# YangHai-1218/RADet

Hardware: AMD Instinct MI355X
Metric: images/sec train-step, r50_ycbv_pbr 640x480 bs=4/GPU (higher is better)
Workload: dtype f32

## Files before the change

include/radet_hip.h:

```cpp
#ifndef RADET_HIP_H
#define RADET_HIP_H
#include <stdint.h>

#ifdef __cplusplus
extern "C" {
#endif


typedef struct RadetConvDesc {
    const float* w;
    const float* bias;
    const float* bn_gamma;
    const float* bn_beta;
    const float* bn_mean;
    const float* bn_var;
    float* wf;
    float* wft;
    float* bias_f;
    const float* dwf_slabs;
    const float* dbias_partials;
    float* dw;
    float* dbias;
    float* dgamma;
    float* dbeta;
// ... 17 lines not shown
    void* y_amax;
    const void* x1_amax;
    const void* w1_amax;
    void* y1_amax;
    void* yq;
    void* yq_amax;
    const void* x_true_amax;
    const void* w_l1;
    const void* bias_amax;
    const void* addend_amax;
} RadetScales;

int radet_gather_table_rows(int M);
int radet_build_gather_table(int* table, int B, int KH, int KW, int so, int sr, int off, int div, const int* seg_desc,
                             int nseg, void* stream);
enum {
    RADET_TILE_ID_MASK = 0xFF,
    RADET_TILE_SYMBOL = 0x100,
    RADET_TILE_BK32 = 0x200,
    RADET_TILE_MATH_BF16 = 0x400,
    RADET_TILE_STORE_BF16 = 0x800,
    RADET_TILE_SPLITK = 0x1000,
    RADET_TILE_SPLITK_MASK = 0xF000,
    RADET_TILE_OUT_F32 = 0x10000,
    RADET_TILE_STAGES3 = 0x20000,
    RADET_TILE_STAGES4 = 0x40000,
    RADET_TILE_ROWPAIRS = 0x80000,
    RADET_TILE_STREAMK = 0x100000,
    RADET_TILE_STREAMK_MASK = 0x700000,
    RADET_TILE_X3 = 0x1000000,
    RADET_TILE_P3 = 0x2000000,
    RADET_TILE_H2 = 0x8000000,
    RADET_TILE_MASKQ = 0x10000000
};
int radet_conv2d_igemm(const float* x, const float* w, const float* bias, const float* addend, const float* mask,
                       float* y, const int* gather_table, int M, int Cin, int Cout, int KH, int KW, int relu,
                       int tile_override, float* splitk_ws, size_t splitk_ws_floats, void* stream);
int radet_conv2d_igemm_s(const float* x, const float* w, const float* bias, const float* addend, const float* mask,
                         float* y, const int* gather_table, int M, int Cin, int Cout, int KH, int KW, int relu,
                         int tile_override, float* splitk_ws, size_t splitk_ws_floats, void* stream, const RadetScales* sc);
int radet_conv2d_igemm_pair_s(const float* x0, const float* w0, const float* bias0, const float* addend0,
                              const float* mask0, float* y0, const float* x1, const float* w1, const float* bias1,
                              const float* addend1, const float* mask1, float* y1, const int* gather_table, int M,
                              int Cin, int Cout, int KH, int KW, int relu, int tile_override, float* splitk_ws,
                              size_t splitk_ws_floats, void* stream, const RadetScales* sc);
int radet_conv2d_igemm_taps_s(const float* x, const float* w, const float* addend, const float* mask, float* y,
                              const int* gather_table, const int* out_rows, const int* tap_ids_host, int ntaps, int kt_w,
                              int M, int Cin, int Cout, int tile_override, float* splitk_ws, size_t splitk_ws_floats,
                              void* stream, const RadetScales* sc);
int radet_conv2d_igemm_classes_s(const float* x, const float* w, const float* addend, const float* mask, float* y,
                                 const int* gather_table, const int* out_rows, const int* tap_ids_host,
                                 const int* cls_ntaps, const int* cls_start, int ncls, int kt_w, int M, int Cin, int Cout,
                                 int tile_override, float* splitk_ws, size_t splitk_ws_floats, void* stream,
                                 const RadetScales* sc);
int radet_conv2d_igemm_pair(const float* x0, const float* w0, const float* bias0, const float* addend0,
                            const float* mask0, float* y0, const float* x1, const float* w1, const float* bias1,
                            const float* addend1, const float* mask1, float* y1, const int* gather_table, int M, int Cin,
                            int Cout, int KH, int KW, int relu, int tile_override, float* splitk_ws,
                            size_t splitk_ws_floats, void* stream);
int radet_conv2d_igemm_taps(const float* x, const float* w, const float* addend, const float* mask, float* y,
                            const int* gather_table, const int* out_rows, const int* tap_ids_host, int ntaps, int kt_w,
                            int M, int Cin, int Cout, int tile_override, float* splitk_ws, size_t splitk_ws_floats,
                            void* stream);
int radet_conv2d_igemm_classes(const float* x, const float* w, const float* addend, const float* mask, float* y,
                               const int* gather_table, const int* out_rows, const int* tap_ids_host, const int* cls_ntaps,
                               const int* cls_start, int ncls, int kt_w, int M, int Cin, int Cout, int tile_override,
// ... 373 lines not shown
```

radet_amd/csrc/common.h:

```cpp
#pragma once
#include <hip/hip_runtime.h>
#include <stdint.h>

#define RADET_MAX_SEG 8

struct RadetSeg {
    int row_end;
    int row_begin;
    int in_row_off;
    int Hi, Wi, Ho, Wo;
};

struct RadetSegs {
    int nseg;
    RadetSeg s[RADET_MAX_SEG];
};

#define RADET_OK 0
#define RADET_ERR_ARG -1
#define RADET_ERR_LAUNCH -2

static inline int radet_check_launch() {
    hipError_t e = hipGetLastError();
    return e == hipSuccess ? RADET_OK : RADET_ERR_LAUNCH;
// ... 1 lines not shown

typedef float f32x16 __attribute__((ext_vector_type(16)));
typedef float f32x4 __attribute__((ext_vector_type(4)));

__device__ __forceinline__ float wave_sum(float v) {
#pragma unroll
    for (int o = 32; o > 0; o >>= 1) v += __shfl_xor(v, o, 64);
    return v;
}
__device__ __forceinline__ double wave_sum_d(double v) {
#pragma unroll
    for (int o = 32; o > 0; o >>= 1) v += __shfl_xor(v, o, 64);
    return v;
}
__device__ __forceinline__ float wave_max(float v) {
#pragma unroll
    for (int o = 32; o > 0; o >>= 1) v = fmaxf(v, __shfl_xor(v, o, 64));
    return v;
}

template <int BYTES>
__device__ __forceinline__ void radet_kernarg_warm() {
    typedef const char __attribute__((address_space(4))) * kptr_t;
    const kptr_t kp = (kptr_t)__builtin_amdgcn_kernarg_segment_ptr();
    constexpr int N = (BYTES + 63) / 64;
    unsigned d[N];
#pragma unroll
    for (int i = 0; i < N; ++i) asm volatile("s_load_dword %0, %1, %2" : "=s"(d[i]) : "s"(kp), "n"(i * 64));
    asm volatile("s_waitcnt lgkmcnt(0)" ::: "memory");
#pragma unroll
    for (int i = 0; i < N; ++i) asm volatile("" ::"s"(d[i]));
}

__device__ __forceinline__ int xcd_remap(int bid, int nwg) {
    const int q = nwg >> 3, r = nwg & 7;
    const int xcd = bid & 7, k = bid >> 3;
    const int base = xcd < r ? xcd * (q + 1) : r * (q + 1) + (xcd - r) * q;
    return base + k;
}

typedef float rd_f32x2 __attribute__((ext_vector_type(2)));
typedef __bf16 rd_bf16x2 __attribute__((ext_vector_type(2)));
__device__ __forceinline__ unsigned radet_pack_bf16(float lo, float hi) {
    const rd_f32x2 v = {lo, hi};
    return __builtin_bit_cast(unsigned, __builtin_convertvector(v, rd_bf16x2));
}
template <class T> __device__ __forceinline__ float4 ld4(const T* p, size_t i4);
template <> __device__ __forceinline__ float4 ld4<float>(const float* p, size_t i4) {
    return reinterpret_cast<const float4*>(p)[i4];
}
template <> __device__ __forceinline__ float4 ld4<__bf16>(const __bf16* p, size_t i4) {
    const uint2 u = reinterpret_cast<const uint2*>(p)[i4];
    return make_float4(__uint_as_float(u.x << 16), __uint_as_float(u.x & 0xFFFF0000u), __uint_as_float(u.y << 16),
                       __uint_as_float(u.y & 0xFFFF0000u));
}
template <class T> __device__ __forceinline__ void st4(T* p, size_t i4, float4 v);
template <> __device__ __forceinline__ void st4<float>(float* p, size_t i4, float4 v) {
    reinterpret_cast<float4*>(p)[i4] = v;
}
template <> __device__ __forceinline__ void st4<__bf16>(__bf16* p, size_t i4, float4 v) {
    reinterpret_cast<uint2*>(p)[i4] = make_uint2(radet_pack_bf16(v.x, v.y), radet_pack_bf16(v.z, v.w));
}

__host__ __device__ __forceinline__ size_t radet_plane_off(int c) {
    return (size_t)(c >> 5) * 96 + (c & 31);
}
__device__ __forceinline__ void radet_split3(const float4 v, uint2& hi, uint2& mid, uint2& lo) {
    const float x[4] = {v.x, v.y, v.z, v.w};
    unsigned h[4], m[4], l[4];
#pragma unroll
    for (int i = 0; i < 4; ++i) {
        h[i] = __float_as_uint(x[i]) & 0xFFFF0000u;
// ... 103 lines not shown
```

radet_amd/csrc/conv_common.h:

```cpp
#pragma once
#include "common.h"
#include "../../include/radet_hip.h"
#include <stdlib.h>
#include <type_traits>

#define RADET_SPLIT_COUNTERS 16384
#ifndef RADET_P3_DBG
#define RADET_P3_DBG 0
#endif

struct ConvPtrs {
    const float* x;
    const float* w;
    const float* bias;
    const float* addend;
    const float* mask;
    float* y;
    const unsigned* xs;
    const unsigned* ws;
    unsigned* ys;
    _Float16* yq;
    unsigned* yqs;
    const unsigned* xt;
    const unsigned* wl1;
    const unsigned* bs;
    const unsigned* as;
};

struct ConvArgs {
    ConvPtrs p[2];
    int groups;
    const int* rowtab;
    float* partial;
    int* counters;
    const int* out_rows;
    int tap_ids[16];
    int KTw;
    int M, Mp, Cin, Cout, KH, KW;
    int relu;
    int sk, it_per_split;
    int n_full, sk_tail, it_per_tail;
    int io;
    int sk_wgs, sk_base, sk_rem;
    int cls_nt, cls_b[3];
    int dbg;
    int maskq;
};

__device__ __forceinline__ float ld_act(const float* p, size_t o, int io) {
    return io ? (float)reinterpret_cast<const __bf16*>(p)[o] : p[o];
}
__device__ __forceinline__ void st_out(float* p, size_t o, float v, int io) {
    if (io == 1) reinterpret_cast<__bf16*>(p)[o] = (__bf16)v;
    else p[o] = v;
}


typedef const __attribute__((address_space(1))) void* gptr_t;
typedef __attribute__((address_space(3))) void* lptr_t;

#ifndef RADET_BUFLDS
#define RADET_BUFLDS 1
#endif
__device__ __forceinline__ __amdgpu_buffer_rsrc_t radet_rsrc(const void* base) {
    return __builtin_amdgcn_make_buffer_rsrc(const_cast<void*>(base), 0, 0xFFFFFF00u, 0x00020000);
}
#if RADET_BUFLDS
#define radet_lds_load16(base, ok, elem_off, dst) \
    __builtin_amdgcn_raw_ptr_buffer_load_lds(radet_rsrc(base), (dst), 16, \
        (int)((ok) ? (unsigned)((elem_off) * sizeof(*(base))) : 0xFFFFFFFFu), 0, 0, 0)
#else
#define radet_lds_load16(base, ok, elem_off, dst) \
    __builtin_amdgcn_global_load_lds((gptr_t)((ok) ? (const void*)((base) + (elem_off)) : (const void*)(radet_zero_page + (threadIdx.x & 63) * 4)), \
                                     (dst), 16, 0, 0)
#endif

__device__ __forceinline__ void radet_pipe_barrier() {
    asm volatile("s_waitcnt lgkmcnt(0)" ::: "memory");
    __builtin_amdgcn_s_barrier();
// ... 417 lines not shown
    acc1 = __builtin_amdgcn_mfma_f32_32x32x16_f16(al, bh, acc1, 0, 0, 0);
}
struct PairScaleRaw { unsigned xt, wl1, bs, as; };
__device__ __forceinline__ PairScaleRaw igemm_pair_scale_load(const ConvPtrs& P) {
    PairScaleRaw r;
    r.xt = radet_amax_load(P.xt); r.wl1 = radet_amax_load(P.wl1);
    r.bs = P.bs ? radet_amax_load(P.bs) : 0u;
    r.as = P.as ? radet_amax_load(P.as) : 0u;
    return r;
}
__device__ __forceinline__ void igemm_pair_scale(const ConvPtrs& P, PairScaleRaw r, bool store, float& qs, float& qs2) {
    asm volatile("" : "+v"(r.xt), "+v"(r.wl1), "+v"(r.bs), "+v"(r.as));
    float bound = __uint_as_float(radet_amax_reduce(r.xt)) * __uint_as_float(radet_amax_reduce(r.wl1));
    bound += __uint_as_float(radet_amax_reduce(r.bs));
    bound += __uint_as_float(radet_amax_reduce(r.as));
    bound *= 1.0001f;
    const unsigned bits = __float_as_uint(bound);
    if (store && threadIdx.x == 0) radet_amax_store(P.yqs, bits);
    const int e = radet_h2_exp(bits);
    qs = radet_pow2(e);
    qs2 = radet_pow2(e + 11);
}

__device__ __forceinline__ void h2_combine(f32x16& acc0, const f32x16& acc1, float inv_a, float inv_b) {
#pragma unroll
    for (int r = 0; r < 16; ++r) acc0[r] = (fmaf(acc1[r], 1.0f / 2048.0f, acc0[r]) * inv_a) * inv_b;
}

struct TileWord {
    int id;
    int splitk;
    int stages;
    int streamk;
    bool symbol, bk32, math_bf16, store_bf16, out_f32, rowpairs, x3, p3, h2, maskq;
};
inline TileWord decode_tile(int t) {
    TileWord r;
    r.id = t & RADET_TILE_ID_MASK;
    r.splitk = (t & RADET_TILE_SPLITK_MASK) / RADET_TILE_SPLITK;
    r.stages = (t & RADET_TILE_STAGES4) ? 4 : ((t & RADET_TILE_STAGES3) ? 3 : 2);
    r.streamk = (t & RADET_TILE_STREAMK_MASK) / RADET_TILE_STREAMK;
    r.symbol = t & RADET_TILE_SYMBOL; r.bk32 = t & RADET_TILE_BK32;
    r.math_bf16 = t & RADET_TILE_MATH_BF16; r.store_bf16 = t & RADET_TILE_STORE_BF16; r.out_f32 = t & RADET_TILE_OUT_F32;
    r.rowpairs = t & RADET_TILE_ROWPAIRS; r.x3 = t & RADET_TILE_X3; r.p3 = t & RADET_TILE_P3; r.h2 = t & RADET_TILE_H2;
    r.maskq = t & RADET_TILE_MASKQ;
    return r;
}
struct WgradFlags {
    int tile;
    bool math_bf16, store_bf16, one_tap, px32, x3, p3, kdiv4, kdiv2, h2, deep, windows;
};
inline WgradFlags decode_wgrad(int f) {
    WgradFlags r;
    r.tile = (f & RADET_WGRAD_TILE_MASK) / RADET_WGRAD_TILE;
    r.math_bf16 = f & RADET_WGRAD_MATH_BF16; r.store_bf16 = f & RADET_WGRAD_STORE_BF16; r.one_tap = f & RADET_WGRAD_ONE_TAP;
    r.px32 = f & RADET_WGRAD_PX32; r.x3 = f & RADET_WGRAD_X3; r.p3 = f & RADET_WGRAD_P3; r.kdiv4 = f & RADET_WGRAD_KDIV4;
    r.kdiv2 = f & RADET_WGRAD_KDIV2; r.h2 = f & RADET_WGRAD_H2; r.deep = f & RADET_WGRAD_DEEP; r.windows = f & RADET_WGRAD_WINDOWS;
    return r;
}

bool radet_launch_igemm_h2(int choice, const ConvArgs& a, hipStream_t st, int tag, int bk, size_t ws_floats, int stages,
                           bool no_tail_split);
struct WgradArgs;
int radet_launch_wgrad_h2(const WgradArgs& a, const WgradFlags& f, int bm, int bn, hipStream_t st);
```

radet_amd/csrc/conv_igemm.hip:

```cpp
#include "common.h"
#include "../../include/radet_hip.h"
#include <stdlib.h>
#include <type_traits>

#include "conv_common.h"

#include "conv_igemm_kernel.h"
#include "conv_wgrad_kernel.h"

struct PredTile { int base_row, H, W, yx; };
struct PredArgs {
    const float* x;
    const float* w[2];
    const float* bias[2];
    float* y[2];
    int c[2];
    const PredTile* tiles;
    int Cin;
};

__global__ __launch_bounds__(512) void pred3x3_patch_kernel(const PredArgs a) {
    constexpr int TH = 8, TW = 16, PW = TW + 2, PP = (TH + 2) * PW;
    constexpr int PROWS = 192, WROWS = 9 * 32;
    constexpr int A_BYTES = PROWS * 64, BUF_BYTES = (PROWS + WROWS) * 64;
// ... 880 lines not shown
    return radet_conv2d_igemm_classes_s(x, w, addend, mask, y, gather_table, out_rows, tap_ids_host, cls_ntaps, cls_start, ncls,
                                        kt_w, M, Cin, Cout, tile_override, splitk_ws, splitk_ws_floats, stream, nullptr);
}

static int igemm_impl(const float* x, const float* w, const float* bias, const float* addend, const float* mask,
                      float* y, const int* gather_table, int M, int Cin, int Cout, int KH, int KW, int relu,
                      int tile_override, float* splitk_ws, size_t splitk_ws_floats, const int* out_rows,
                      const int* tap_ids, int kt_w, void* stream, const ConvPtrs* second, const int* cls,
                      const RadetScales* sc) {
    const TileWord tw = decode_tile(tile_override);
    const bool h16 = tw.store_bf16;
    const bool p3 = tw.p3 && !h16;
    if (h16 || p3) {
        if (Cin % 32 != 0) return RADET_ERR_ARG;
        Cin /= 2;
    }
    if (Cin % 16 != 0 || Cin <= 0 || Cout <= 0 || M <= 0 || KH * KW > 16 ||
        (gather_table == nullptr && (KH * KW != 1 || out_rows != nullptr || cls != nullptr)))
        return RADET_ERR_ARG;
    ConvArgs a;
    a.io = h16 ? (tw.out_f32 ? 2 : 1) : 0;
    a.out_rows = out_rows;
    for (int t = 0; t < 16; ++t) a.tap_ids[t] = tap_ids ? (t < KH * KW ? tap_ids[t] : 0) : t;
    a.cls_nt = 0; a.cls_b[0] = a.cls_b[1] = a.cls_b[2] = 0x7fffffff;
    if (cls != nullptr) {
        for (int t = 0; t < 16; ++t) a.tap_ids[t] = tap_ids[t];
        for (int c = 0; c < cls[0]; ++c) {
            a.cls_nt |= cls[1 + c] << (4 * c);
            if (c > 0) a.cls_b[c - 1] = cls[5 + c];
        }
    }
    a.KTw = kt_w > 0 ? kt_w : KH * KW;
    { static const int dbg = getenv("RADET_DBG_IGEMM") ? atoi(getenv("RADET_DBG_IGEMM")) : 0; a.dbg = dbg; }
    a.maskq = tw.maskq && mask != nullptr;
    if (a.maskq && (h16 || Cout % 32 != 0 || second != nullptr)) return RADET_ERR_ARG;
    if (y == nullptr && (sc == nullptr || sc->yq == nullptr)) return RADET_ERR_ARG;
    a.p[0].x = x; a.p[0].w = w; a.p[0].bias = bias; a.p[0].addend = addend; a.p[0].mask = mask; a.p[0].y = y;
    a.p[0].xs = sc ? (const unsigned*)sc->x_amax : nullptr;
    a.p[0].ws = sc ? (const unsigned*)sc->w_amax : nullptr;
    a.p[0].ys = sc ? (unsigned*)sc->y_amax : nullptr;
    a.p[0].yq = sc ? (_Float16*)sc->yq : nullptr;
    a.p[0].yqs = sc ? (unsigned*)sc->yq_amax : nullptr;
    a.p[0].xt = sc ? (const unsigned*)sc->x_true_amax : nullptr;
    a.p[0].wl1 = sc ? (const unsigned*)sc->w_l1 : nullptr;
    a.p[0].bs = (sc && bias) ? (const unsigned*)sc->bias_amax : nullptr;
    a.p[0].as = (sc && addend) ? (const unsigned*)sc->addend_amax : nullptr;
    if (a.p[0].yq != nullptr) {
        if (h16 || Cout % 32 != 0 || a.p[0].yqs == nullptr || a.p[0].xt == nullptr || a.p[0].wl1 == nullptr ||
            (bias && a.p[0].bs == nullptr) || (addend && a.p[0].as == nullptr) || second != nullptr)
            return RADET_ERR_ARG;
    }
    a.p[1] = a.p[0];
    a.groups = 1;
    if (second != nullptr) {
        a.p[1] = *second;
        a.p[1].yq = nullptr; a.p[1].yqs = nullptr; a.p[1].xt = a.p[1].wl1 = a.p[1].bs = a.p[1].as = nullptr;
        a.p[1].xs = sc ? (const unsigned*)sc->x1_amax : nullptr;
        a.p[1].ws = sc ? (const unsigned*)sc->w1_amax : nullptr;
        a.p[1].ys = sc ? (unsigned*)sc->y1_amax : nullptr;
        a.groups = 2;
    }
    a.rowtab = gather_table;
    a.Cin = Cin; a.Cout = Cout; a.KH = KH; a.KW = KW;
    a.relu = relu;
    a.M = M;
    a.Mp = radet_gather_table_rows(M);
// ... 154 lines not shown
    return (int)S;
}

static int wgrad_impl(const float* dy, const float* x, float* slabs, float* dbias_partials, const int* gather_table, int M,
                      int Cin, int Cout, int ld_dy, int KH, int KW, int S, int flags, void* stream, const RadetScales* sc);
extern "C" int radet_conv2d_wgrad(const float* dy, const float* x, float* slabs, float* dbias_partials,
                                  const int* gather_table, int M, int Cin, int Cout, int ld_dy, int KH, int KW, int S,
                                  int flags, void* stream) {
    return wgrad_impl(dy, x, slabs, dbias_partials, gather_table, M, Cin, Cout, ld_dy, KH, KW, S, flags, stream, nullptr);
}
extern "C" int radet_conv2d_wgrad_s(const float* dy, const float* x, float* slabs, float* dbias_partials,
                                    const int* gather_table, int M, int Cin, int Cout, int ld_dy, int KH, int KW, int S,
                                    int flags, void* stream, const RadetScales* sc) {
    return wgrad_impl(dy, x, slabs, dbias_partials, gather_table, M, Cin, Cout, ld_dy, KH, KW, S, flags, stream, sc);
}
static int wgrad_impl(const float* dy, const float* x, float* slabs, float* dbias_partials, const int* gather_table, int M,
                      int Cin, int Cout, int ld_dy, int KH, int KW, int S, int flags, void* stream, const RadetScales* sc) {
    if (Cin % 4 != 0 || S < 1 || ld_dy < Cout || (ld_dy & 3) || ((Cout + 3) / 4) * 4 > ld_dy || M <= 0 ||
        (gather_table == nullptr && KH * KW != 1))
        return RADET_ERR_ARG;
    const WgradFlags f = decode_wgrad(flags);
    if (f.store_bf16 && ((Cout + 7) / 8) * 8 > ld_dy) return RADET_ERR_ARG;
    WgradArgs a;
    a.ld_dy = ld_dy;
    a.dy = dy; a.x = x; a.slabs = slabs; a.dbias_partials = dbias_partials;
    a.rowtab = gather_table;
    a.Cin = Cin; a.Cout = Cout; a.KH = KH; a.KW = KW;
    a.M = M;
    a.Mp = radet_gather_table_rows(M);
    a.S = S;
    a.dbg = radet_switches().dbg_wgrad;
    a.math = f.math_bf16 ? 1 : (f.x3 && !f.store_bf16 ? 2 : 0);
    a.bp32 = f.px32;
    a.dys = sc ? (const unsigned*)sc->x_amax : nullptr;
    a.xss = sc ? (const unsigned*)sc->w_amax : nullptr;
    const int chunks = (a.M + 15) / 16;
    a.chunks_per_split = (chunks + S - 1) / S;
    hipStream_t st = (hipStream_t)stream;
    if (f.h2) {
        if (f.math_bf16 || f.store_bf16 || a.dys == nullptr || a.xss == nullptr) return RADET_ERR_ARG;
        a.math = 3;
        int bm = 0, bn = 0;
        if (!f.p3) wgrad_onetap_tile(f, true, M, Cout, Cin, KH * KW, &bm, &bn);
        return radet_launch_wgrad_h2(a, f, bm, bn, st);
    }
    if (f.p3) {
        if ((ld_dy & 31) || (Cin & 31) || f.math_bf16 || f.store_bf16) return RADET_ERR_ARG;
        if (KH == 3 && KW == 3 && Cin % 32 == 0) {
            const int tiles9 = ((Cout + 255) / 256) * (Cin / 32) * S;
            hipLaunchKernelGGL(conv_wgrad9p_kernel, dim3(tiles9), dim3(512), 0, st, a);
            return radet_check_launch();
        }
        return RADET_ERR_ARG;
    }
    if (f.store_bf16) {
        if ((ld_dy & 7) || (Cin & 7)) return RADET_ERR_ARG;
        if (use_wgrad9(M, Cin, Cout, KH, KW) && wgrad9_bm(Cout) == 256 && !f.one_tap && !radet_switches().no_wgrad9) {
            const int tiles9 = ((Cout + 255) / 256) * (Cin / 32) * S;
            hipLaunchKernelGGL(conv_wgrad9h_kernel, dim3(tiles9), dim3(512), 0, st, a);
            return radet_check_launch();
        }
        int bm, bn;
        wgrad_onetap_tile(f, false, M, Cout, Cin, KH * KW, &bm, &bn);
        const int tiles = ((Cout + bm - 1) / bm) * ((Cin + bn - 1) / bn) * KH * KW * S;
        if (bm == 32) hipLaunchKernelGGL((conv_wgradh_kernel<32, 128, 1, 4>), dim3(tiles), dim3(256), 0, st, a);
        else if (bm == 64) hipLaunchKernelGGL((conv_wgradh_kernel<64, 64, 2, 2>), dim3(tiles), dim3(256), 0, st, a);
// ... 14 lines not shown
    }
    int bm, bn;
    wgrad_onetap_tile(f, a.math == 2, M, Cout, Cin, KH * KW, &bm, &bn);
    if (bm == 64 && a.math == 2 && (f.kdiv4 || f.kdiv2)) {
        const int tiles = ((a.Cout + 63) / 64) * ((a.Cin + 63) / 64) * a.KH * a.KW * a.S;
        if (f.kdiv4) hipLaunchKernelGGL((conv_wgradg_kernel<64, 64, 2, 2, 2, 64, 4>), dim3(tiles), dim3(256), 0, st, a);
        else hipLaunchKernelGGL((conv_wgradg_kernel<64, 64, 2, 2, 2, 32, 2>), dim3(tiles), dim3(256), 0, st, a);
    } else
    if (bm == 32) launch_wgrad<32, 128, 1, 4>(a, st);
    else if (bm == 64) launch_wgrad<64, 64, 2, 2>(a, st);
    else if (bn == 64) {
        const int tiles = ((a.Cout + 127) / 128) * ((a.Cin + 63) / 64) * a.KH * a.KW * a.S;
        if (a.bp32) hipLaunchKernelGGL((conv_wgradg_kernel<128, 64, 2, 2, 2, 32>), dim3(tiles), dim3(256), 0, st, a);
        else hipLaunchKernelGGL((conv_wgradg_kernel<128, 64, 2, 2, 2>), dim3(tiles), dim3(256), 0, st, a);
    } else launch_wgrad<128, 128, 2, 2>(a, st);
    return radet_check_launch();
}

extern "C" int radet_conv2d_wgrad_group(const RadetWgradJob* jobs, int njobs, int flags, void* stream) {
    if (njobs < 1 || njobs > WG_MAX || jobs == nullptr) return RADET_ERR_ARG;
    const WgradFlags f = decode_wgrad(flags);
    const int bm = f.tile == 1 ? 128 : 64;
    WgradGroup g;
    g.n = njobs;
    int total = 0;
    for (int i = 0; i < njobs; ++i) {
        const RadetWgradJob& j = jobs[i];
        if (j.Cin % 4 != 0 || j.S < 1 || j.ld_dy < j.Cout || (j.ld_dy & 3) || j.M <= 0 || (j.gather_table == nullptr && j.KH * j.KW != 1) ||
            j.Cout % bm != 0 || j.Cin % bm != 0)
            return RADET_ERR_ARG;
        WgradArgs& a = g.p[i];
        a.dy = j.dy; a.x = j.x; a.slabs = j.slabs; a.dbias_partials = j.dbias_partials; a.rowtab = j.gather_table;
        a.M = j.M; a.Mp = radet_gather_table_rows(j.M); a.Cin = j.Cin; a.Cout = j.Cout; a.KH = j.KH; a.KW = j.KW;
        a.ld_dy = j.ld_dy; a.S = j.S; a.dbg = 0; a.math = f.math_bf16; a.bp32 = 0; a.dys = a.xss = nullptr;
        const int chunks = (j.M + 15) / 16;
        a.chunks_per_split = (chunks + j.S - 1) / j.S;
        g.begin[i] = total;
        total += (j.Cout / bm) * (j.Cin / bm) * j.KH * j.KW * j.S;
    }
    g.begin[njobs] = total;
    hipStream_t st = (hipStream_t)stream;
    if (bm == 128) {
        if (f.math_bf16) hipLaunchKernelGGL((conv_wgradg_group_kernel<128, 128, 2, 2, 1>), dim3(total), dim3(256), 0, st, g);
        else hipLaunchKernelGGL((conv_wgradg_group_kernel<128, 128, 2, 2, 0>), dim3(total), dim3(256), 0, st, g);
    } else {
        if (f.math_bf16) hipLaunchKernelGGL((conv_wgradg_group_kernel<64, 64, 2, 2, 1>), dim3(total), dim3(256), 0, st, g);
        else hipLaunchKernelGGL((conv_wgradg_group_kernel<64, 64, 2, 2, 0>), dim3(total), dim3(256), 0, st, g);
    }
    return radet_check_launch();
}
```

radet_amd/csrc/conv_igemm_kernel.h:

```cpp
#pragma once
#include "conv_common.h"
static __device__ __attribute__((aligned(16))) float radet_zero_page[512];

constexpr int TAG_SYMBOL = 1;
constexpr int TAG_BF16_MATH = 2;
constexpr int TAG_H16 = 4;
constexpr int TAG_X3 = 8;
constexpr int TAG_P3 = 16;
constexpr int TAG_KDIV = 32;
constexpr int TAG_H2 = 64;
constexpr int TAG_PAIRS = 128;
template <int BM, int BN, int WM, int WN, int TAG, int BK, int NSTG = 2, bool SK = false>
__global__ __launch_bounds__(WM * WN * 64) void conv_igemmg_kernel(const ConvArgs a) {
    constexpr int NW = WM * WN;
    constexpr int F4 = BK / 4;
    constexpr int RPI = 64 / F4;
    constexpr int RPB = 64 / BK;
    constexpr int TM = BM / (WM * 32), TN = BN / (WN * 32);
    constexpr int A_INSTR = BM / RPI, B_INSTR = BN / RPI;
    constexpr int A_PW = (A_INSTR + NW - 1) / NW, B_PW = (B_INSTR + NW - 1) / NW;
    constexpr int NS = ((TAG & TAG_PAIRS) && (TAG & TAG_P3)) ? 2 : BK / 8;
    constexpr bool BF16 = (TAG & TAG_BF16_MATH) != 0;
    constexpr bool H16 = (TAG & TAG_H16) != 0;
    constexpr bool X3 = (TAG & TAG_X3) != 0;
// ... 8 lines not shown
    constexpr bool PQ = (TAG & TAG_PAIRS) != 0 && (TAG & TAG_KDIV) != 0;
    static_assert(!PQ || (KW && H2 && BK == 64), "pair operands in the K-divided tile: 64-channel stages");
    constexpr int KD = KW ? BK / 16 : 1;
    constexpr int WNK = NW / KD;
    constexpr int TMA = KW ? BM / 32 : TM, TNA = KW ? BN / (32 * WNK) : TN;
    static_assert(!KW || (X3 && !SK && NW == 4 && KD * WNK == NW && TM == 1 && TN == 1 && TMA * TNA == KD && NSTG >= 2 && NSTG <= 4),
                  "K-divided tile: one 32 x 32 block per wave after the reduction");
    static_assert(NW == 4 || NW == 8, "4 or 8 waves");
    static_assert(!P3 || BK == 16 || RI, "plane rows are laid out in 32-channel groups: one group per K stage");
    __shared__ __attribute__((aligned(16))) float As[NSTG][NPL * BM * BK];
    __shared__ __attribute__((aligned(16))) float Bs[NSTG][NPL * BN * BK];

    radet_kernarg_warm<sizeof(ConvArgs)>();
    const int tid = threadIdx.x;
    const int lane = tid & 63, wave = __builtin_amdgcn_readfirstlane(tid >> 6);
    const int wm = wave / WN, wn = wave % WN;
    const int li = lane & 31, lh = lane >> 5;
    const int xld = NPL * a.Cin;

    const int tilesN = (a.Cout + BN - 1) / BN;
    const int tilesG = ((a.M + BM - 1) / BM) * tilesN;
    const int KT = a.KH * a.KW;
    const int cpt = a.Cin / BK;
    constexpr bool streamk = SK;
    const int vwg = streamk ? ((int)blockIdx.x & 7) * (a.sk_wgs >> 3) + ((int)blockIdx.x >> 3) : 0;
    int cur = streamk ? streamk_start(a, vwg) : 0;
    const int end_it = streamk ? cur + a.sk_base + (vwg < a.sk_rem ? 1 : 0) : 1;
    const int first_tile = cur / (KT * cpt);
  do {
    const bool tail = !streamk && (int)blockIdx.x >= a.n_full;
    const int tail_slot = tail ? (int)blockIdx.x - a.n_full : 0;
    int id = streamk ? cur / (KT * cpt)
                     : (tail ? a.n_full + tail_slot / a.sk_tail : (a.cls_nt ? (int)blockIdx.x : xcd_remap(blockIdx.x, a.n_full)));
    const int sk_tile = id;
    const int grp = id >= tilesG ? 1 : 0;
    id -= grp * tilesG;
    ConvPtrs P = a.p[grp];
    P.y = pin_sgpr(P.y); P.bias = pin_sgpr(P.bias); P.addend = pin_sgpr(P.addend); P.mask = pin_sgpr(P.mask);
    EpiArgs epi;
    epi.M = pin_sgpr(a.M); epi.Cout = pin_sgpr(a.Cout); epi.relu = pin_sgpr(a.relu); epi.io = pin_sgpr(a.io);
    epi.out_rows = pin_sgpr(a.out_rows); epi.maskq = pin_sgpr(a.maskq);
    epi.partial = pin_sgpr(a.partial); epi.counters = pin_sgpr(a.counters);
    epi.sk_base = pin_sgpr(a.sk_base); epi.sk_rem = pin_sgpr(a.sk_rem);
    epi.qs = 1.f; epi.qs2 = 2048.f;
    unsigned raw_xs = 0u, raw_ws = 0u;
    if constexpr ((TAG & TAG_H2) != 0) { raw_xs = h2_scale_load(P.xs); raw_ws = h2_scale_load(P.ws); }
    PairScaleRaw raw_q = {0u, 0u, 0u, 0u};
    const bool pair_copy = P.yq != nullptr;
    if (pair_copy) raw_q = igemm_pair_scale_load(P);
    const bool pair_store = id == 0 && (int)blockIdx.y == 0 && !SK;
    const int nsplit = pin_sgpr(tail ? a.sk_tail : a.sk);
    const int ctile = pin_sgpr(tail ? tail_slot / a.sk_tail : sk_tile);
    const int zsplit = pin_sgpr(tail ? tail_slot % a.sk_tail : (int)blockIdx.y);
    const int m0 = (id / tilesN) * BM;
    const int n0 = (id % tilesN) * BN;
    int KTt = KT, tbase = 0;
    if (!streamk && a.cls_nt) {
        const int cls = (m0 >= a.cls_b[0] ? 1 : 0) + (m0 >= a.cls_b[1] ? 1 : 0) + (m0 >= a.cls_b[2] ? 1 : 0);
        KTt = (a.cls_nt >> (4 * cls)) & 15;
        tbase = 4 * cls;
    }

    const int per = tail ? a.it_per_tail : a.it_per_split;
    const int it0 = streamk ? cur - sk_tile * KT * cpt : (tail ? tail_slot % a.sk_tail : (int)blockIdx.y) * per;
    int nK = KTt * cpt - it0;
    if (streamk) {
// ... 554 lines not shown
    const int T = a.groups * ((a.M + BM - 1) / BM) * ((a.Cout + BN - 1) / BN);
    a.sk_wgs = a.sk_base = a.sk_rem = 0;
    if (skw > 0 && a.partial != nullptr && tag == 0 && BM * BN <= 128 * 64) {
        const long I = (long)T * a.KH * a.KW * (a.Cin / bk);
        const int G = 256 * skw;
        if (I >= G && T <= RADET_SPLIT_COUNTERS && (size_t)G * 2 * BM * BN <= ws_floats && T % G != 0) {
            a.sk = 1;
            a.it_per_split = a.KH * a.KW * (a.Cin / bk);
            a.sk_wgs = G;
            a.sk_base = (int)(I / G);
            a.sk_rem = (int)(I % G);
        }
    }
    while (a.sk > 1 && ((size_t)T * a.sk * BM * BN > ws_floats || T > RADET_SPLIT_COUNTERS)) --a.sk;
    if (a.sk != sk_in) {
        const int nKs0 = a.KH * a.KW * (a.Cin / bk);
        a.it_per_split = (nKs0 + a.sk - 1) / a.sk;
    }
    a.n_full = T; a.sk_tail = 1; a.it_per_tail = a.it_per_split;
    const int nKs = a.KH * a.KW * (a.Cin / bk);
    const int rem = T % 256;
    if (a.sk_wgs == 0 && a.cls_nt == 0 && a.sk == 1 && a.partial != nullptr && T > 256 && rem > 0 && rem <= 160 && nKs * bk >= 512 &&
        !no_tail_split) {
        int skt = 256 / rem;
        if (skt > 8) skt = 8;
        if (skt > nKs / 8) skt = nKs / 8;
        while (skt > 1 && ((size_t)rem * skt * BM * BN > ws_floats || rem > RADET_SPLIT_COUNTERS)) --skt;
        if (skt >= 2) {
            a.n_full = T - rem;
            a.sk_tail = skt;
            a.it_per_tail = (nKs + skt - 1) / skt;
        }
    }
    return a.sk_wgs > 0 ? a.sk_wgs : a.n_full + (T - a.n_full) * a.sk_tail;
}
```

radet_amd/csrc/conv_wgrad_h2.hip:

```cpp
#include "common.h"
#include "../../include/radet_hip.h"
#include <stdlib.h>
#include <type_traits>

#include "conv_igemm_kernel.h"
#include "conv_wgrad_kernel.h"

#if RADET_P3_DBG
__device__ long long radet_dbg_clk[2][64][4];
extern "C" int radet_dbg_clk_read(long long* host, int n) {
    return (int)hipMemcpyFromSymbol(host, HIP_SYMBOL(radet_dbg_clk), (size_t)n * sizeof(long long));
}
#define RADET_STAMP(it, pt) do { if (blockIdx.x == 0 && (wave == 0 || wave == 4) && (it) < 64) { \
    const long long t_ = __builtin_amdgcn_s_memtime(); asm volatile("s_waitcnt lgkmcnt(0)" ::: "memory"); \
    if (lane == 0) radet_dbg_clk[wave >> 2][(it)][(pt)] = t_; } } while (0)
#else
#define RADET_STAMP(it, pt) do { } while (0)
#endif
template <int SUB, bool SPREAD = false, bool TGLOAD = false>
__global__ __launch_bounds__(512) void conv_wgrad9q_kernel(const WgradArgs a) {
    radet_kernarg_warm<sizeof(WgradArgs)>();
    constexpr int BP = 16, NW = 8, BM = 128, BC = 32, KT = 9;
    constexpr int CBA = BM / 16, CBB = BC / 16;
    constexpr int A_PL = BP * BM, B_PL = BP * BC;
// ... 605 lines not shown
                const int o = o0 + og * 32 + (r & 3) + 8 * (r >> 2) + 4 * lh;
                if (o < a.Cout) out[((size_t)o * KT + tap0 + t) * a.Cin + c] = acc[t][r];
            }
        }
    }
}

template <int BM, int BN, int WM, int WN>
__global__ __launch_bounds__(256) void conv_wgradq_kernel(const WgradArgs a) {
    radet_kernarg_warm<sizeof(WgradArgs)>();
    constexpr int BP = 32, NW = 4;
    constexpr int TM = BM / (WM * 32), TN = BN / (WN * 32);
    constexpr int CBA = BM / 16, CBB = BN / 16;
    constexpr int A_PL = BP * BM, B_PL = BP * BN;
    constexpr int A_Q = A_PL * 2 / 1024, B_Q = B_PL * 2 / 1024;
    constexpr int A_INSTR = 2 * A_Q, B_INSTR = 2 * B_Q;
    constexpr int N_INSTR = A_INSTR + B_INSTR;
    constexpr int PER_WAVE = (N_INSTR + NW - 1) / NW;
    static_assert(WM * WN == 4, "4 waves");
    __shared__ __attribute__((aligned(16))) unsigned short As[2][2 * A_PL];
    __shared__ __attribute__((aligned(16))) unsigned short Bs[2][2 * B_PL];
    const unsigned short* dyh = reinterpret_cast<const unsigned short*>(a.dy);
    const unsigned short* xh = reinterpret_cast<const unsigned short*>(a.x);

    const int tid = threadIdx.x;
    const int lane = tid & 63, wave = __builtin_amdgcn_readfirstlane(tid >> 6);
    const int wm = wave / WN, wn = wave % WN;
    const int li = lane & 31, lh = lane >> 5;

    const int KT = a.KH * a.KW;
    const int tilesO = (a.Cout + BM - 1) / BM;
    const int tilesC = (a.Cin + BN - 1) / BN;
    const int tilesPerSplit = tilesO * tilesC * KT;
    int id = blockIdx.x;
    const int split = id / tilesPerSplit;
    id -= split * tilesPerSplit;
    const int to = id % tilesO;
    id /= tilesO;
    const int tc = id % tilesC;
    const int tap = id / tilesC;
    const int o0 = to * BM, c0 = tc * BN;
    const int* tab_tap = a.rowtab ? a.rowtab + (size_t)tap * a.Mp : nullptr;

    const int p_begin = split * a.chunks_per_split * 16;
    int p_end = p_begin + a.chunks_per_split * 16;
    if (p_end > a.M) p_end = a.M;
    const int nIt = p_begin < p_end ? (p_end - p_begin + BP - 1) / BP : 0;

    const int l_blk = lane >> 3, l_prow = (lane & 7) >> 1, l_half = lane & 1;
    int brow[PER_WAVE];
    bool bok[PER_WAVE];
#pragma unroll
    for (int k = 0; k < PER_WAVE; ++k) {
        const int bi = wave + k * NW - A_INSTR;
        brow[k] = -1;
        bok[k] = false;
        if (bi >= 0 && bi < B_INSTR) {
            const int blk = (bi % B_Q) * 8 + l_blk;
            const int m = p_begin + 4 * (blk / CBB) + l_prow;
            brow[k] = tab_tap ? tab_tap[m < a.Mp ? m : a.Mp - 1] : m;
            bok[k] = m < p_end;
        }
    }
    auto issue_stage = [&](int it, int buf) {
#pragma unroll
        for (int k = 0; k < PER_WAVE; ++k) asm volatile("" : "+v"(brow[k]));
        const int p0 = p_begin + it * BP;
// ... 184 lines not shown
```

radet_amd/csrc/conv_wgrad_kernel.h:

```cpp
#pragma once
#include "conv_igemm_kernel.h"
struct WgradArgs {
    const float* dy;
    const float* x;
    float* slabs;
    float* dbias_partials;
    const int* rowtab;
    int M, Mp, Cin, Cout, KH, KW;
    int ld_dy;
    int S;
    int chunks_per_split;
    int dbg;
    int math;
    int bp32;
    const unsigned* dys;
    const unsigned* xss;
};



template <int NW, int MATH>
__global__ __launch_bounds__(NW * 64) void conv_wgrad9g_kernel(const WgradArgs a) {
    radet_kernarg_warm<sizeof(WgradArgs)>();
    constexpr int BP = 16, BM = 32 * NW, BC = 32, KT = 9, NT = NW * 64;
    constexpr int A_INSTR = BP * BM * 4 / 1024;
    constexpr int B_INSTR = KT * BP * BC * 4 / 1024;
    constexpr int N_INSTR = A_INSTR + B_INSTR;
    constexpr int PER_WAVE = (N_INSTR + NW - 1) / NW;
    constexpr int ROWS_A = 1024 / (BM * 4);
    __shared__ __attribute__((aligned(16))) float As[2][BP * BM];
    __shared__ __attribute__((aligned(16))) float Bs[2][KT * BP * BC];

    const int tid = threadIdx.x;
    const int lane = tid & 63, wave = __builtin_amdgcn_readfirstlane(tid >> 6);
    const int li = lane & 31, lh = lane >> 5;

    const int tilesO = (a.Cout + BM - 1) / BM;
    const int tilesC = a.Cin / BC;
    const int tilesPerSplit = tilesO * tilesC;
    int id = blockIdx.x;
    const int split = id / tilesPerSplit;
    id -= split * tilesPerSplit;
    const int to = id % tilesO, tc = id / tilesO;
    const int o0 = to * BM, c0 = tc * BC;

    const int p_begin = split * a.chunks_per_split * BP;
    int p_end = p_begin + a.chunks_per_split * BP;
    if (p_end > a.M) p_end = a.M;
    const int nIt = p_begin < p_end ? (p_end - p_begin + BP - 1) / BP : 0;
// ... 500 lines not shown
                    const f32x4 t = d[q * 64];
                    res[4 * q] += t.x; res[4 * q + 1] += t.y; res[4 * q + 2] += t.z; res[4 * q + 3] += t.w;
                }
            }
        }
        const int c = c0 + (nh * TNA + kg % TNA) * 32 + li;
        if (c < a.Cin) {
#pragma unroll
            for (int t = 0; t < 16; ++t) {
                const int o = o0 + (kg / TNA) * 32 + (t & 3) + 8 * (t >> 2) + 4 * lh;
                if (o < a.Cout) out[((size_t)o * KT + tap) * a.Cin + c] = res[t];
            }
        }
    } else {
#pragma unroll
    for (int i = 0; i < TM; ++i)
#pragma unroll
        for (int j = 0; j < TN; ++j) {
            const int c = c0 + (wn * TN + j) * 32 + li;
            if (c >= a.Cin) continue;
#pragma unroll
            for (int t = 0; t < 16; ++t) {
                const int o = o0 + (wm * TM + i) * 32 + (t & 3) + 8 * (t >> 2) + 4 * lh;
                if (o >= a.Cout) continue;
                out[((size_t)o * KT + tap) * a.Cin + c] = acc[i][j][t];
            }
        }
    }
}

template <int BM, int BN, int WM, int WN, int MATH, int BP = 16, int KD = 1>
__global__ __launch_bounds__(256) void conv_wgradg_kernel(const WgradArgs a) {
    radet_kernarg_warm<sizeof(WgradArgs)>();
    wgradg_body<BM, BN, WM, WN, MATH, BP, KD>(a, blockIdx.x);
}

#define WG_MAX 32
struct WgradGroup {
    int n;
    int begin[WG_MAX + 1];
    WgradArgs p[WG_MAX];
};

template <int BM, int BN, int WM, int WN, int MATH>
__global__ __launch_bounds__(256) void conv_wgradg_group_kernel(const WgradGroup g) {
    int pi = 0;
    for (int i = 1; i < g.n; ++i)
        if ((int)blockIdx.x >= g.begin[i]) pi = i;
    wgradg_body<BM, BN, WM, WN, MATH>(g.p[pi], (int)blockIdx.x - g.begin[pi]);
}
```

radet_amd/kernels.py:

```python
import ctypes as C
import os

import torch

from . import _lib

ID_MASK = 0xFF
SYMBOL = 0x100
BK32 = 0x200
MATH_BF16 = 0x400
STORE_BF16, OUT_F32 = 0x800, 0x10000
SPLITK, SPLITK_MASK = 0x1000, 0xF000
STAGES3 = 0x20000
STAGES4 = 0x40000
ROWPAIRS = 0x80000
STREAMK, STREAMK_MASK = 0x100000, 0x700000
X3 = 0x1000000
P3 = 0x2000000
H2 = 0x8000000
MASKQ = 0x10000000
WG_MATH_BF16, WG_STORE_BF16 = 0x1, 0x2
WG_TILE, WG_TILE_MASK = 0x10, 0x30
WG_ONE_TAP = 0x40
WG_PX32 = 0x80
WG_X3 = 0x100
WG_P3 = 0x200
WG_KDIV4, WG_KDIV2 = 0x400, 0x800
WG_H2 = 0x1000
WG_DEEP, WG_WINDOWS = 0x2000, 0x4000
TAG_SYMBOL, TAG_BF16_MATH, TAG_H16, TAG_X3, TAG_P3, TAG_KDIV, TAG_H2, TAG_PAIRS = 1, 2, 4, 8, 16, 32, 64, 128

TILE_SHAPE = {1: (128, 128), 2: (128, 64), 3: (64, 64), 4: (128, 32), 5: (128, 128), 6: (256, 128), 7: (64, 64), 8: (64, 64)}
WG_TILE_SHAPE = {1: (128, 128), 2: (64, 64), 3: (128, 64)}


def splitk(n):
    return n * SPLITK


def streamk(w):
    return w * STREAMK


def tile_id(t):
    return t & ID_MASK


def with_tile(t, tid):
    return (t & ~(ID_MASK | SPLITK_MASK)) | tid


def wg_tile(flags):
    return (flags & WG_TILE_MASK) // WG_TILE



def _ptr(t):
    if t is None:
        return None
    if not (t.is_cuda and t.is_contiguous()):
        raise AssertionError("HIP kernels need contiguous device tensors")
    return t.data_ptr()

# ... 1723 lines not shown
```

Baseline: 500.0.

## Add XCD-aware grouped tile ordering for igemm and wgrad grids

Adds a grid_order helper that reorders igemm output tiles into column groups sized to the eight XCDs. A cost model over weight and activation bytes picks the group width, aiming to improve L2 reuse of weights and inputs within each XCD. Wgrad kernels now apply xcd_remap to block ids by default, with a flag bit to keep the old linear order. This changes tile-to-CU mapping, so it may also change load balance and streaming behaviour.

```diff
diff --git a/include/radet_hip.h b/include/radet_hip.h
--- a/include/radet_hip.h
+++ b/include/radet_hip.h
@@ -73,6 +73,10 @@
     RADET_TILE_P3 = 0x2000000,
     RADET_TILE_H2 = 0x8000000,
     RADET_TILE_MASKQ = 0x10000000
+};
+enum {
+    RADET_GRID_ORDER_TILE = 0x4000000,
+    RADET_GRID_ORDER_WGRAD = 0x8000
 };
 int radet_conv2d_igemm(const float* x, const float* w, const float* bias, const float* addend, const float* mask,
                        float* y, const int* gather_table, int M, int Cin, int Cout, int KH, int KW, int relu,
diff --git a/radet_amd/csrc/common.h b/radet_amd/csrc/common.h
--- a/radet_amd/csrc/common.h
+++ b/radet_amd/csrc/common.h
@@ -57,12 +57,7 @@
     for (int i = 0; i < N; ++i) asm volatile("" ::"s"(d[i]));
 }
 
-__device__ __forceinline__ int xcd_remap(int bid, int nwg) {
-    const int q = nwg >> 3, r = nwg & 7;
-    const int xcd = bid & 7, k = bid >> 3;
-    const int base = xcd < r ? xcd * (q + 1) : r * (q + 1) + (xcd - r) * q;
-    return base + k;
-}
+#include "grid_order.h"
 
 typedef float rd_f32x2 __attribute__((ext_vector_type(2)));
 typedef __bf16 rd_bf16x2 __attribute__((ext_vector_type(2)));
diff --git a/radet_amd/csrc/conv_common.h b/radet_amd/csrc/conv_common.h
--- a/radet_amd/csrc/conv_common.h
+++ b/radet_amd/csrc/conv_common.h
@@ -45,6 +45,7 @@
     int cls_nt, cls_b[3];
     int dbg;
     int maskq;
+    int gn;
 };
 
 __device__ __forceinline__ float ld_act(const float* p, size_t o, int io) {
@@ -528,7 +529,7 @@
     int splitk;
     int stages;
     int streamk;
-    bool symbol, bk32, math_bf16, store_bf16, out_f32, rowpairs, x3, p3, h2, maskq;
+    bool symbol, bk32, math_bf16, store_bf16, out_f32, rowpairs, x3, p3, h2, maskq, grid_order;
 };
 inline TileWord decode_tile(int t) {
     TileWord r;
@@ -539,12 +540,12 @@
     r.symbol = t & RADET_TILE_SYMBOL; r.bk32 = t & RADET_TILE_BK32;
     r.math_bf16 = t & RADET_TILE_MATH_BF16; r.store_bf16 = t & RADET_TILE_STORE_BF16; r.out_f32 = t & RADET_TILE_OUT_F32;
     r.rowpairs = t & RADET_TILE_ROWPAIRS; r.x3 = t & RADET_TILE_X3; r.p3 = t & RADET_TILE_P3; r.h2 = t & RADET_TILE_H2;
-    r.maskq = t & RADET_TILE_MASKQ;
+    r.maskq = t & RADET_TILE_MASKQ; r.grid_order = t & RADET_GRID_ORDER_TILE;
     return r;
 }
 struct WgradFlags {
     int tile;
-    bool math_bf16, store_bf16, one_tap, px32, x3, p3, kdiv4, kdiv2, h2, deep, windows;
+    bool math_bf16, store_bf16, one_tap, px32, x3, p3, kdiv4, kdiv2, h2, deep, windows, grid_order;
 };
 inline WgradFlags decode_wgrad(int f) {
     WgradFlags r;
@@ -552,6 +553,7 @@
     r.math_bf16 = f & RADET_WGRAD_MATH_BF16; r.store_bf16 = f & RADET_WGRAD_STORE_BF16; r.one_tap = f & RADET_WGRAD_ONE_TAP;
     r.px32 = f & RADET_WGRAD_PX32; r.x3 = f & RADET_WGRAD_X3; r.p3 = f & RADET_WGRAD_P3; r.kdiv4 = f & RADET_WGRAD_KDIV4;
     r.kdiv2 = f & RADET_WGRAD_KDIV2; r.h2 = f & RADET_WGRAD_H2; r.deep = f & RADET_WGRAD_DEEP; r.windows = f & RADET_WGRAD_WINDOWS;
+    r.grid_order = f & RADET_GRID_ORDER_WGRAD;
     return r;
 }
 
diff --git a/radet_amd/csrc/conv_igemm.hip b/radet_amd/csrc/conv_igemm.hip
--- a/radet_amd/csrc/conv_igemm.hip
+++ b/radet_amd/csrc/conv_igemm.hip
@@ -936,6 +936,7 @@
     }
     a.KTw = kt_w > 0 ? kt_w : KH * KW;
     { static const int dbg = getenv("RADET_DBG_IGEMM") ? atoi(getenv("RADET_DBG_IGEMM")) : 0; a.dbg = dbg; }
+    a.gn = tw.grid_order ? 1 : 0;
     a.maskq = tw.maskq && mask != nullptr;
     if (a.maskq && (h16 || Cout % 32 != 0 || second != nullptr)) return RADET_ERR_ARG;
     if (y == nullptr && (sc == nullptr || sc->yq == nullptr)) return RADET_ERR_ARG;
@@ -1156,6 +1157,7 @@
     a.dbg = radet_switches().dbg_wgrad;
     a.math = f.math_bf16 ? 1 : (f.x3 && !f.store_bf16 ? 2 : 0);
     a.bp32 = f.px32;
+    a.grid_order = f.grid_order;
     a.dys = sc ? (const unsigned*)sc->x_amax : nullptr;
     a.xss = sc ? (const unsigned*)sc->w_amax : nullptr;
     const int chunks = (a.M + 15) / 16;
@@ -1236,7 +1238,7 @@
         WgradArgs& a = g.p[i];
         a.dy = j.dy; a.x = j.x; a.slabs = j.slabs; a.dbias_partials = j.dbias_partials; a.rowtab = j.gather_table;
         a.M = j.M; a.Mp = radet_gather_table_rows(j.M); a.Cin = j.Cin; a.Cout = j.Cout; a.KH = j.KH; a.KW = j.KW;
-        a.ld_dy = j.ld_dy; a.S = j.S; a.dbg = 0; a.math = f.math_bf16; a.bp32 = 0; a.dys = a.xss = nullptr;
+        a.ld_dy = j.ld_dy; a.S = j.S; a.dbg = 0; a.math = f.math_bf16; a.bp32 = 0; a.dys = a.xss = nullptr; a.grid_order = 0;
         const int chunks = (j.M + 15) / 16;
         a.chunks_per_split = (chunks + j.S - 1) / j.S;
         g.begin[i] = total;
diff --git a/radet_amd/csrc/conv_igemm_kernel.h b/radet_amd/csrc/conv_igemm_kernel.h
--- a/radet_amd/csrc/conv_igemm_kernel.h
+++ b/radet_amd/csrc/conv_igemm_kernel.h
@@ -64,6 +64,11 @@
     const int tail_slot = tail ? (int)blockIdx.x - a.n_full : 0;
     int id = streamk ? cur / (KT * cpt)
                      : (tail ? a.n_full + tail_slot / a.sk_tail : (a.cls_nt ? (int)blockIdx.x : xcd_remap(blockIdx.x, a.n_full)));
+    if (!streamk && a.gn > 1) {
+        int tm, tn;
+        tile_order_2d(id, tilesG / tilesN, tilesN, a.gn, &tm, &tn);
+        id = tm * tilesN + tn;
+    }
     const int sk_tile = id;
     const int grp = id >= tilesG ? 1 : 0;
     id -= grp * tilesG;
@@ -684,5 +689,11 @@
             a.it_per_tail = (nKs + skt - 1) / skt;
         }
     }
+    if (a.gn == 0 && a.groups == 1 && a.cls_nt == 0 && a.sk_wgs == 0 && a.n_full == T) {
+        const long long w_bytes = 4ll * a.Cout * a.KH * a.KW * a.Cin, x_bytes = 4ll * a.M * a.Cin;
+        a.gn = igemm_pick_gn((a.M + BM - 1) / BM, (a.Cout + BN - 1) / BN, w_bytes, x_bytes);
+    } else {
+        a.gn = 1;
+    }
     return a.sk_wgs > 0 ? a.sk_wgs : a.n_full + (T - a.n_full) * a.sk_tail;
 }
diff --git a/radet_amd/csrc/conv_wgrad_h2.hip b/radet_amd/csrc/conv_wgrad_h2.hip
--- a/radet_amd/csrc/conv_wgrad_h2.hip
+++ b/radet_amd/csrc/conv_wgrad_h2.hip
@@ -661,7 +661,7 @@
     const int tilesO = (a.Cout + BM - 1) / BM;
     const int tilesC = (a.Cin + BN - 1) / BN;
     const int tilesPerSplit = tilesO * tilesC * KT;
-    int id = blockIdx.x;
+    int id = a.grid_order ? (int)blockIdx.x : xcd_remap((int)blockIdx.x, (int)gridDim.x);
     const int split = id / tilesPerSplit;
     id -= split * tilesPerSplit;
     const int to = id % tilesO;
diff --git a/radet_amd/csrc/conv_wgrad_kernel.h b/radet_amd/csrc/conv_wgrad_kernel.h
--- a/radet_amd/csrc/conv_wgrad_kernel.h
+++ b/radet_amd/csrc/conv_wgrad_kernel.h
@@ -15,6 +15,7 @@
     int bp32;
     const unsigned* dys;
     const unsigned* xss;
+    int grid_order;
 };
 
 
@@ -581,7 +582,7 @@
 template <int BM, int BN, int WM, int WN, int MATH, int BP = 16, int KD = 1>
 __global__ __launch_bounds__(256) void conv_wgradg_kernel(const WgradArgs a) {
     radet_kernarg_warm<sizeof(WgradArgs)>();
-    wgradg_body<BM, BN, WM, WN, MATH, BP, KD>(a, blockIdx.x);
+    wgradg_body<BM, BN, WM, WN, MATH, BP, KD>(a, a.grid_order ? (int)blockIdx.x : xcd_remap((int)blockIdx.x, (int)gridDim.x));
 }
 
 #define WG_MAX 32
diff --git a/radet_amd/csrc/grid_order.h b/radet_amd/csrc/grid_order.h
--- /dev/null
+++ b/radet_amd/csrc/grid_order.h
@@ -0,0 +1,54 @@
+#pragma once
+#if defined(__HIPCC__)
+#define RADET_HD __host__ __device__ __forceinline__
+#else
+#define RADET_HD inline
+#endif
+
+RADET_HD int xcd_remap(int bid, int nwg) {
+    const int q = nwg >> 3, r = nwg & 7;
+    const int xcd = bid & 7, k = bid >> 3;
+    const int base = xcd < r ? xcd * (q + 1) : r * (q + 1) + (xcd - r) * q;
+    return base + k;
+}
+
+RADET_HD void grid_group_of(int j, int n, int g, int stride, int* first, int* size) {
+    const int q = n / g, r = n - q * g;
+    const int big = r * (q + 1) * stride;
+    int grp;
+    if (j < big) {
+        grp = j / ((q + 1) * stride);
+        *size = q + 1;
+    } else {
+        grp = r + (j - big) / (q * stride);
+        *size = q;
+    }
+    *first = grp * q + (grp < r ? grp : r);
+}
+
+RADET_HD void tile_order_2d(int j, int tilesM, int tilesN, int gN, int* tm, int* tn) {
+    if (gN <= 1) {
+        *tm = j / tilesN;
+        *tn = j - *tm * tilesN;
+        return;
+    }
+    int col0, w, row0, h;
+    grid_group_of(j, tilesN, gN, tilesM, &col0, &w);
+    j -= col0 * tilesM;
+    grid_group_of(j, tilesM, 8 / gN, w, &row0, &h);
+    j -= row0 * w;
+    const int r = j / w;
+    *tm = row0 + r;
+    *tn = col0 + (j - r * w);
+}
+
+RADET_HD int igemm_pick_gn(int tilesM, int tilesN, long long w_bytes, long long x_bytes) {
+    int best = 1;
+    long long best_cost = 8 * w_bytes + x_bytes;
+    for (int g = 2; g <= 8; g *= 2) {
+        if (g > tilesN || 8 / g > tilesM) continue;
+        const long long cost = (8 / g) * w_bytes + g * x_bytes;
+        if (cost < best_cost) { best_cost = cost; best = g; }
+    }
+    return best;
+}
diff --git a/radet_amd/kernels.py b/radet_amd/kernels.py
--- a/radet_amd/kernels.py
+++ b/radet_amd/kernels.py
@@ -29,6 +29,8 @@
 WG_H2 = 0x1000
 WG_DEEP, WG_WINDOWS = 0x2000, 0x4000
 TAG_SYMBOL, TAG_BF16_MATH, TAG_H16, TAG_X3, TAG_P3, TAG_KDIV, TAG_H2, TAG_PAIRS = 1, 2, 4, 8, 16, 32, 64, 128
+GRID_ORDER_TILE = 0x4000000
+GRID_ORDER_WGRAD = 0x8000
 
 TILE_SHAPE = {1: (128, 128), 2: (128, 64), 3: (64, 64), 4: (128, 32), 5: (128, 128), 6: (256, 128), 7: (64, 64), 8: (64, 64)}
 WG_TILE_SHAPE = {1: (128, 128), 2: (64, 64), 3: (128, 64)}
```

Measured after the change: 500.0 (median of 4 runs). No clear change (+0.0%).
